# ollieeknight/mgatk2

Measured on AMD Instinct MI355X. Metric: chrM reads piled-up/sec (whole node) at 200M reads × 10k cells; bit-exact counts, higher is better.
Workload: dtype u32

## Files before the change

include/mgpileup.h:

```cpp
#ifndef MGPILEUP_H
#define MGPILEUP_H

#include <stdint.h>

#ifdef __cplusplus
extern "C" {
#endif

#define MGP_ABI_VERSION 7

#define MGP_OK               0
#define MGP_E_INVALID      (-1)
#define MGP_E_HIP          (-2)
#define MGP_E_OOM          (-3)
#define MGP_E_UNSORTED     (-4)
#define MGP_E_BADREAD      (-5)
#define MGP_E_SPAN         (-6)
#define MGP_E_STATE        (-7)
#define MGP_E_COMM         (-8)

#define MGP_DEDUP_NONE        0
#define MGP_DEDUP_START       1
#define MGP_DEDUP_START_FRAG  2

// ... 404 lines not shown
int  mgp_louvain(int device, int64_t n_vertices, int64_t n_edges, const int32_t *edge_i, const int32_t *edge_j,
                 const int32_t *edge_w, double resolution, int32_t max_levels, int32_t max_passes,
                 int32_t *labels , int64_t *n_communities, double *modularity,
                 uint64_t *sums , int32_t *n_levels, int64_t *levels );
int  mgp_windows(mgp_ctx *ctx, int32_t *n_windows, int32_t *window_width);
int  mgp_copy_wait(mgp_ctx *ctx);
int  mgp_set_cell_range(mgp_ctx *ctx, int32_t cell_lo, int32_t cell_hi);
int  mgp_push_batch16(mgp_ctx *ctx, const mgp_batch16 *batch);
int  mgp_set_streaming(mgp_ctx *ctx, int on);
int  mgp_stream_info(mgp_ctx *ctx, int64_t *segments, int32_t *last_streamed);
int  mgp_finish(mgp_ctx *ctx, mgp_result *out);

int  mgp_kernel_times(mgp_ctx *ctx, int last_runs, float *ms, int max_n, int *n_out, char *names, int names_len);
int  mgp_set_stage_timing(mgp_ctx *ctx, int all_stages);

int  mgp_comm_unique_id(uint8_t *out128);
int  mgp_comm_init(mgp_ctx *ctx, const uint8_t *uid128, int nranks, int rank);

int  mgp_synth_generate(mgp_ctx *ctx, const mgp_synth_params *p);
int  mgp_download_inputs(mgp_ctx *ctx, int32_t *start, int32_t *bc, int32_t *tlen,
                         uint16_t *flag, uint8_t *mapq, uint32_t *span,
                         uint64_t *rec_off, uint8_t *payload);

int  mgp_bgzf_inflate(int device, const uint8_t *src, int64_t src_bytes, int64_t n_blocks,
                      const uint64_t *coff, const uint32_t *clen, const uint32_t *isize, const uint64_t *out_off,
                      uint8_t *out, int64_t out_bytes, int32_t *status );
typedef struct mgp_inflater mgp_inflater;
int  mgp_inflater_create(int device, int64_t max_src_bytes, int64_t max_out_bytes, mgp_inflater **out);
void mgp_inflater_destroy(mgp_inflater *inflater);
int  mgp_inflater_run(void *inflater, const uint8_t *src, int64_t src_bytes, int64_t n_blocks,
                      const uint64_t *coff, const uint32_t *clen, const uint32_t *isize, const uint64_t *out_off,
                      uint8_t *out, int64_t out_bytes, int32_t *status);
int  mgp_inflater_times(mgp_inflater *inflater, double *ms3, int64_t *calls, int64_t *blocks);
void *mgp_inflater_host_alloc(int64_t bytes);
void  mgp_inflater_host_release(void *p);

int  mgp_zlib_inflate(int device, const uint8_t *src, int64_t src_bytes, int64_t n_streams,
                      const uint64_t *coff, const uint32_t *clen, const uint32_t *isize, const uint64_t *out_off,
                      uint8_t *out, int64_t out_bytes, int32_t *status );
int  mgp_open_table(int hip_device, int32_t n_cells, int32_t mito_len, mgp_ctx **out);
typedef struct mgp_table_chunks {
    int64_t        n_cols;
    int32_t        chunk_rows, chunk_cols;
    int32_t        col_chunk_lo, col_chunk_hi;
    int32_t        first_cell;
    int32_t        reserved;
    const uint8_t *src;
    int64_t        src_bytes;
    const int64_t *chunk_bytes;
    const uint8_t *raw;
    int64_t        n_saturated;
    double         ms[3];
} mgp_table_chunks;
int  mgp_table_load(mgp_ctx *table, mgp_table_chunks *job);
int  mgp_table_load_planes(mgp_ctx *table, mgp_table_chunks *job);
int  mgp_table_check(int32_t n_cells, int32_t mito_len, const mgp_table_chunks *job, int planes);
int  mgp_table_ready(mgp_ctx *table);

#ifdef __cplusplus
}
#endif
#endif
```

mgatk2_amd/csrc/mgp_inflate.hip:

```cpp
#include <hip/hip_runtime.h>

#include <cstring>
#include <string>
#include <vector>

#include "../../include/mgpileup.h"
#include "mgp_host.h"
#include "mgp_inflate_core.h"

namespace {

using namespace mgp_inflate;

struct DeviceWave {
    __device__ uint32_t lane() const { return threadIdx.x; }
    __device__ uint32_t width() const { return 64; }
    __device__ bool leader() const { return threadIdx.x == 0; }
    __device__ void sync() const { __syncthreads(); }
};

__global__ __launch_bounds__(64) void inflate_blocks(const uint8_t* __restrict__ src, const uint64_t* __restrict__ coff,
                                                     const uint32_t* __restrict__ clen,
                                                     const uint32_t* __restrict__ isize,
                                                     const uint64_t* __restrict__ out_off, uint8_t* __restrict__ out,
                                                     int32_t* __restrict__ status, uint32_t n_blocks) {
    __shared__ Scratch sc;
    __shared__ alignas(16) uint8_t win[kMaxIsize];
    const uint32_t b = blockIdx.x;
    if (b >= n_blocks) return;
    const DeviceWave w;
    const uint32_t n = isize[b];
    const int32_t st = inflate(w, src + coff[b], clen[b], win, n, &sc);
    if (st == ST_OK) flush(w, win, n, out + out_off[b]);
    if (w.leader()) status[b] = st;
}

struct Args {
    const uint8_t* src;
    int64_t src_bytes, n_blocks;
    const uint64_t* coff;
    const uint32_t* clen;
    const uint32_t* isize;
    const uint64_t* out_off;
    uint8_t* out;
    int64_t out_bytes;
    int32_t* status;
};

int check_args(const char* who, const Args& a) {
    const std::string w(who);
    if (a.n_blocks < 0 || a.src_bytes < 0 || a.out_bytes < 0) return set_err(MGP_E_INVALID, w + ": negative count");
    if (a.n_blocks > 0x7FFFFFFF) return set_err(MGP_E_INVALID, w + ": more than 2^31 - 1 blocks in one call");
    if (a.n_blocks && (!a.coff || !a.clen || !a.isize || !a.out_off || !a.status))
        return set_err(MGP_E_INVALID, w + ": null array");
    if ((a.src_bytes && !a.src) || (a.out_bytes && !a.out)) return set_err(MGP_E_INVALID, w + ": null buffer");
    uint64_t end = 0;
    for (int64_t i = 0; i < a.n_blocks; ++i) {
        const std::string at = " (block " + std::to_string(i) + ")";
        if (a.isize[i] > kMaxIsize) return set_err(MGP_E_INVALID, w + ": isize above 65536" + at);
        if (a.coff[i] > (uint64_t)a.src_bytes || a.clen[i] > (uint64_t)a.src_bytes - a.coff[i])
            return set_err(MGP_E_INVALID, w + ": compressed range outside src" + at);
        if (a.out_off[i] > (uint64_t)a.out_bytes || a.isize[i] > (uint64_t)a.out_bytes - a.out_off[i])
            return set_err(MGP_E_INVALID, w + ": output range outside out" + at);
        if (a.out_off[i] < end) return set_err(MGP_E_INVALID, w + ": output ranges unsorted or overlapping" + at);
        end = a.out_off[i] + a.isize[i];
    }
// ... 125 lines not shown
    if (inf->s) (void)hipStreamSynchronize(inf->s);
    delete inf;
}

int mgp_inflater_run(void* inflater, const uint8_t* src, int64_t src_bytes, int64_t n_blocks, const uint64_t* coff,
                     const uint32_t* clen, const uint32_t* isize, const uint64_t* out_off, uint8_t* out,
                     int64_t out_bytes, int32_t* status) {
    if (!inflater) return set_err(MGP_E_INVALID, "mgp_inflater_run: null inflater");
    const Args a{src, src_bytes, n_blocks, coff, clen, isize, out_off, out, out_bytes, status};
    return inflater_run(static_cast<mgp_inflater*>(inflater), "mgp_inflater_run", a);
}

int mgp_bgzf_inflate(int device, const uint8_t* src, int64_t src_bytes, int64_t n_blocks, const uint64_t* coff,
                     const uint32_t* clen, const uint32_t* isize, const uint64_t* out_off, uint8_t* out,
                     int64_t out_bytes, int32_t* status) {
    const Args a{src, src_bytes, n_blocks, coff, clen, isize, out_off, out, out_bytes, status};
    MGP_TRY(check_args("mgp_bgzf_inflate", a));
    if (n_blocks == 0) return MGP_OK;
    mgp_inflater* inf = nullptr;
    MGP_TRY(inflater_create(device, src_bytes, out_bytes, &inf));
    const int rc = inflater_run(inf, "mgp_bgzf_inflate", a);
    mgp_inflater_destroy(inf);
    return rc;
}

int mgp_inflater_times(mgp_inflater* inf, double* ms3, int64_t* calls, int64_t* blocks) {
    if (!inf || !ms3) return set_err(MGP_E_INVALID, "mgp_inflater_times: null argument");
    for (int k = 0; k < 3; ++k) ms3[k] = inf->ms[k];
    if (calls) *calls = inf->calls;
    if (blocks) *blocks = inf->blocks;
    return MGP_OK;
}

void* mgp_inflater_host_alloc(int64_t bytes) {
    void* p = nullptr;
    return mgp_host_alloc(bytes, &p) == MGP_OK ? p : nullptr;
}
void mgp_inflater_host_release(void* p) { (void)mgp_host_free(p); }

}
```

mgatk2_amd/csrc/mgp_inflate_core.h:

```cpp
#pragma once
#include <stdint.h>

#if defined(__HIPCC__) || defined(__CUDACC__)
#define MGPI_HD __host__ __device__
#else
#define MGPI_HD
#endif

namespace mgp_inflate {

enum : int32_t { ST_OK = 0, ST_INVALID = 1, ST_SIZE = 2, ST_CHECK = 3 };

constexpr uint32_t kMaxIsize = 65536;
constexpr uint32_t kRing = 65536, kHalf = 32768;
constexpr uint32_t kAdlerMod = 65521;
constexpr uint32_t kMaxLanes = 64;
constexpr uint32_t kInWin = 4096;
constexpr uint32_t kLitBits = 10, kDistBits = 8, kClBits = 7;
constexpr uint32_t kMaxLit = 288, kMaxDist = 32, kMaxCl = 19;

struct Huff {
    uint16_t count[16];
    uint16_t first[16];
    uint16_t offs[16];
    uint16_t sorted[kMaxLit];
};

struct Scratch {
    alignas(16) uint8_t inwin[kInWin];
    uint16_t lit_tab[1u << kLitBits];
    uint16_t dist_tab[1u << kDistBits];
    uint16_t cl_tab[1u << kClBits];
    Huff lit, dist, cl;
    uint8_t lens[kMaxLit + kMaxDist];
    uint8_t cl_lens[kMaxCl + 1];
    uint32_t red[2 * kMaxLanes];
};

struct HostWave {
    MGPI_HD uint32_t lane() const { return 0; }
    MGPI_HD uint32_t width() const { return 1; }
    MGPI_HD bool leader() const { return true; }
    MGPI_HD void sync() const {}
};

struct Bits {
    const uint8_t* src;
    uint32_t clen;
    uint64_t bitbuf = 0;
    uint32_t bitcnt = 0;
    uint32_t ip = 0;
    uint32_t wbase = 0, wend = 0;
};

template <class W>
MGPI_HD inline void fill_window(const W& w, Bits& b, Scratch* s) {
    w.sync();
    b.wbase = b.ip;
    b.wend = b.ip + kInWin;
    for (uint32_t i = w.lane(); i < kInWin; i += w.width()) {
        const uint32_t g = b.wbase + i;
        s->inwin[i] = g < b.clen ? b.src[g] : (uint8_t)0;
    }
    w.sync();
}

template <class W>
MGPI_HD inline void refill(const W& w, Bits& b, Scratch* s) {
    for (int k = 0; k < 2; ++k) {
        if (b.bitcnt > 32 || b.ip >= b.clen) return;
        if (b.ip >= b.wend) fill_window(w, b, s);
        const uint32_t o = b.ip - b.wbase;
        const uint32_t word = (uint32_t)s->inwin[o] | (uint32_t)s->inwin[o + 1] << 8 | (uint32_t)s->inwin[o + 2] << 16 |
                              (uint32_t)s->inwin[o + 3] << 24;
        const uint32_t left = b.clen - b.ip;
        const uint32_t nb = left < 4 ? left : 4;
        b.bitbuf |= (uint64_t)word << b.bitcnt;
        b.bitcnt += 8 * nb;
        b.ip += nb;
    }
}

MGPI_HD inline uint32_t peek(const Bits& b, uint32_t n) { return (uint32_t)(b.bitbuf & ((1ull << n) - 1)); }
MGPI_HD inline void drop(Bits& b, uint32_t n) {
    b.bitbuf >>= n;
    b.bitcnt -= n;
}

MGPI_HD inline uint32_t bitrev(uint32_t v, uint32_t n) {
    uint32_t r = 0;
    for (uint32_t i = 0; i < 15; ++i) {
        if (i < n) r |= ((v >> i) & 1u) << (n - 1 - i);
    }
    return r;
}

template <class W>
MGPI_HD inline int32_t build(const W& w, const uint8_t* lens, uint32_t nsym, uint32_t cap, bool is_codes, Huff* h,
                             uint16_t* tab, uint32_t bits) {
    if (nsym > cap) nsym = cap;
    const uint32_t tsize = 1u << bits;
    w.sync();
    for (uint32_t l = w.lane(); l < 16; l += w.width()) {
        uint32_t c = 0;
        for (uint32_t i = 0; i < nsym; ++i) c += (lens[i] & 15u) == l;
        h->count[l] = (uint16_t)c;
    }
    for (uint32_t i = w.lane(); i < tsize; i += w.width()) tab[i] = 0;
    w.sync();
    uint32_t maxlen = 0;
    int32_t left = 1;
    bool over = false;
    for (uint32_t l = 1; l < 16; ++l) {
        const uint32_t c = h->count[l];
        if (c) maxlen = l;
        left <<= 1;
        left -= (int32_t)c;
        if (left < 0) {
            over = true;
            left = 0;
        }
    }
    if (over) return ST_INVALID;
    if (maxlen == 0) return is_codes ? ST_INVALID : ST_OK;
    if (left > 0 && (is_codes || maxlen != 1)) return ST_INVALID;
    if (w.leader()) {
        uint32_t code = 0, off = 0;
        h->first[0] = 0;
        h->offs[0] = 0;
        for (uint32_t l = 1; l < 16; ++l) {
            code = (code + h->count[l - 1] * (l > 1)) << 1;
            h->first[l] = (uint16_t)code;
            h->offs[l] = (uint16_t)off;
            off += h->count[l];
        }
    }
    w.sync();
    for (uint32_t l = 1 + w.lane(); l < 16; l += w.width()) {
        uint32_t k = h->offs[l];
        const uint32_t end = k + h->count[l];
        for (uint32_t i = 0; i < nsym; ++i)
            if ((lens[i] & 15u) == l && k < end && k < kMaxLit) h->sorted[k++] = (uint16_t)i;
    }
    w.sync();
    const uint32_t nused = nsym - h->count[0];
    for (uint32_t j = w.lane(); j < nused && j < kMaxLit; j += w.width()) {
        const uint32_t sym = h->sorted[j];
        const uint32_t l = sym < nsym ? (lens[sym] & 15u) : 0;
        if (l == 0 || l > bits) continue;
        const uint32_t code = (uint32_t)h->first[l] + (j - h->offs[l]);
        const uint16_t e = (uint16_t)(sym << 4 | l);
        for (uint32_t k = bitrev(code, l) & (tsize - 1); k < tsize; k += 1u << l) tab[k] = e;
    }
    w.sync();
    return ST_OK;
}

MGPI_HD inline int32_t decode(const Bits& b, const Huff* h, const uint16_t* tab, uint32_t bits, uint32_t* sym,
                              uint32_t* len) {
    const uint32_t e = tab[peek(b, bits)];
    if (e & 15u) {
        *sym = e >> 4;
        *len = e & 15u;
        return ST_OK;
    }
    uint32_t code = 0, first = 0, index = 0;
    uint64_t v = b.bitbuf;
    for (uint32_t l = 1; l < 16; ++l) {
        code |= (uint32_t)(v & 1);
        v >>= 1;
        const uint32_t c = h->count[l];
        if (code < first + c) {
            const uint32_t k = index + (code - first);
            if (k >= kMaxLit) return ST_INVALID;
            *sym = h->sorted[k];
            *len = l;
            return ST_OK;
        }
        index += c;
        first = (first + c) << 1;
        code <<= 1;
    }
    return ST_INVALID;
}

MGPI_HD inline uint32_t len_base(uint32_t s) {
    return s < 8 ? 3 + s : s == 28 ? 258 : 3 + ((4 + (s & 3)) << ((s >> 2) - 1));
}
MGPI_HD inline uint32_t len_extra(uint32_t s) { return s < 8 || s == 28 ? 0 : (s >> 2) - 1; }
MGPI_HD inline uint32_t dist_base(uint32_t s) {
    return s < 4 ? 1 + s : 1 + ((2 + (s & 1)) << ((s >> 1) - 1));
}
MGPI_HD inline uint32_t dist_extra(uint32_t s) { return s < 4 ? 0 : (s >> 1) - 1; }

template <class W>
MGPI_HD inline void fixed_lens(const W& w, Scratch* s) {
    w.sync();
    for (uint32_t i = w.lane(); i < kMaxLit + kMaxDist; i += w.width())
        s->lens[i] = (uint8_t)(i < 144 ? 8 : i < 256 ? 9 : i < 280 ? 7 : i < 288 ? 8 : 5);
}

template <class W>
MGPI_HD inline int32_t dynamic_header(const W& w, Bits& b, Scratch* s, uint32_t* nlen_out, uint32_t* ndist_out) {
    constexpr uint64_t order_lo = 16ull | 17ull << 5 | 18ull << 10 | 0ull << 15 | 8ull << 20 | 7ull << 25 | 9ull << 30 |
                                  6ull << 35 | 10ull << 40 | 5ull << 45 | 11ull << 50 | 4ull << 55;
    constexpr uint64_t order_hi = 12ull | 3ull << 5 | 13ull << 10 | 2ull << 15 | 14ull << 20 | 1ull << 25 | 15ull << 30;
    refill(w, b, s);
    if (b.bitcnt < 14) return ST_SIZE;
    const uint32_t nlen = peek(b, 5) + 257;
    drop(b, 5);
    const uint32_t ndist = peek(b, 5) + 1;
    drop(b, 5);
    const uint32_t ncode = peek(b, 4) + 4;
    drop(b, 4);
    if (nlen > 286 || ndist > 30) return ST_INVALID;
    w.sync();
    for (uint32_t i = 0; i < kMaxCl; ++i) {
        uint32_t v = 0;
        if (i < ncode) {
            refill(w, b, s);
            if (b.bitcnt < 3) return ST_SIZE;
            v = peek(b, 3);
            drop(b, 3);
        }
        const uint32_t at = (uint32_t)((i < 12 ? order_lo >> (5 * i) : order_hi >> (5 * (i - 12))) & 31u);
        if (w.leader() && at < kMaxCl) s->cl_lens[at] = (uint8_t)v;
    }
    int32_t rc = build(w, s->cl_lens, kMaxCl, kMaxCl, true, &s->cl, s->cl_tab, kClBits);
    if (rc != ST_OK) return rc;
    const uint32_t total = nlen + ndist;
    uint32_t have = 0, prev = 0;
    for (uint32_t step = 0; step < kMaxLit + kMaxDist && have < total; ++step) {
        refill(w, b, s);
        uint32_t sym, len;
        if (decode(b, &s->cl, s->cl_tab, kClBits, &sym, &len) != ST_OK) return ST_INVALID;
        if (len > b.bitcnt) return ST_SIZE;
        drop(b, len);
        uint32_t rep = 1, val = sym;
        if (sym >= 16) {
            const uint32_t eb = sym == 16 ? 2 : sym == 17 ? 3 : 7;
            if (sym > 18) return ST_INVALID;
            if (b.bitcnt < eb) return ST_SIZE;
            if (sym == 16 && have == 0) return ST_INVALID;
            rep = (sym == 16 ? 3 : sym == 17 ? 3 : 11) + peek(b, eb);
            drop(b, eb);
            val = sym == 16 ? prev : 0;
            if (have + rep > total) return ST_INVALID;
        }
        if (w.leader())
            for (uint32_t k = 0; k < rep; ++k) {
                const uint32_t i = have + k;
                const uint32_t at = i < nlen ? i : kMaxLit + (i - nlen);
                if (at < kMaxLit + kMaxDist) s->lens[at] = (uint8_t)val;
            }
        have += rep;
        prev = val;
    }
    if (have != total) return ST_INVALID;
    w.sync();
    if (s->lens[256] == 0) return ST_INVALID;
    *nlen_out = nlen;
    *ndist_out = ndist;
    return ST_OK;
}

template <class W>
MGPI_HD inline int32_t inflate(const W& w, const uint8_t* src, uint32_t clen, uint8_t* win, uint32_t isize, Scratch* s) {
    if (isize > kMaxIsize || clen >= 0x80000000u) return ST_INVALID;
    Bits b;
    b.src = src;
    b.clen = clen;
    uint32_t op = 0;
    uint64_t budget = 8ull * clen + 64;
    bool final_seen = false;
    while (!final_seen) {
        if (budget-- == 0) return ST_INVALID;
        refill(w, b, s);
        if (b.bitcnt < 3) return ST_SIZE;
        final_seen = peek(b, 1) != 0;
        const uint32_t type = peek(b, 3) >> 1;
        drop(b, 3);
        if (type == 3) return ST_INVALID;
        if (type == 0) {
            drop(b, b.bitcnt & 7);
            refill(w, b, s);
            if (b.bitcnt < 32) return ST_SIZE;
            const uint32_t len = peek(b, 16);
            drop(b, 16);
            const uint32_t nlen = peek(b, 16);
            drop(b, 16);
            if ((len ^ 0xFFFFu) != nlen) return ST_INVALID;
            const uint32_t pos = b.ip - (b.bitcnt >> 3);
            if (len > clen - pos) return ST_SIZE;
            if (len > isize - op) return ST_SIZE;
            w.sync();
            for (uint32_t i = w.lane(); i < len; i += w.width()) win[op + i] = src[pos + i];
            w.sync();
            op += len;
            b.bitbuf = 0;
            b.bitcnt = 0;
            b.ip = pos + len;
            b.wbase = b.wend = b.ip;
            continue;
        }
        uint32_t nlen = kMaxLit, ndist = kMaxDist;
        if (type == 1) {
            fixed_lens(w, s);
        } else {
            const int32_t rc = dynamic_header(w, b, s, &nlen, &ndist);
            if (rc != ST_OK) return rc;
        }
        int32_t rc = build(w, s->lens, nlen, kMaxLit, false, &s->lit, s->lit_tab, kLitBits);
        if (rc != ST_OK) return rc;
        rc = build(w, s->lens + kMaxLit, ndist, kMaxDist, false, &s->dist, s->dist_tab, kDistBits);
        if (rc != ST_OK) return rc;
        bool end_of_block = false;
        while (!end_of_block) {
            if (budget-- == 0) return ST_INVALID;
            refill(w, b, s);
            uint32_t sym, len;
            if (decode(b, &s->lit, s->lit_tab, kLitBits, &sym, &len) != ST_OK) return ST_INVALID;
            if (len > b.bitcnt) return ST_SIZE;
            drop(b, len);
            if (sym < 256) {
                if (op >= isize) return ST_SIZE;
                if (w.leader()) win[op] = (uint8_t)sym;
                ++op;
                continue;
            }
            if (sym == 256) {
                end_of_block = true;
                continue;
            }
            if (sym >= 286) return ST_INVALID;
            const uint32_t ls = sym - 257;
            const uint32_t le = len_extra(ls);
            if (b.bitcnt < le) return ST_SIZE;
            const uint32_t mlen = len_base(ls) + peek(b, le);
            drop(b, le);
            refill(w, b, s);
            uint32_t dsym, dlen;
            if (decode(b, &s->dist, s->dist_tab, kDistBits, &dsym, &dlen) != ST_OK) return ST_INVALID;
            if (dlen > b.bitcnt) return ST_SIZE;
            drop(b, dlen);
            if (dsym >= 30) return ST_INVALID;
            const uint32_t de = dist_extra(dsym);
            if (b.bitcnt < de) return ST_SIZE;
            const uint32_t dist = dist_base(dsym) + peek(b, de);
            drop(b, de);
            if (dist > op) return ST_INVALID;
            if (mlen > isize - op) return ST_SIZE;
            w.sync();
            const uint32_t from = op - dist;
            if (dist >= mlen) {
                for (uint32_t i = w.lane(); i < mlen; i += w.width()) win[op + i] = win[from + i];
            } else {
                for (uint32_t i = w.lane(); i < mlen; i += w.width()) win[op + i] = win[from + i % dist];
            }
            w.sync();
            op += mlen;
        }
    }
    w.sync();
    return op == isize ? ST_OK : ST_SIZE;
}

template <class W>
MGPI_HD inline void flush(const W& w, const uint8_t* win, uint32_t n, uint8_t* dst) {
    const uint32_t mis = (uint32_t)((4u - ((uintptr_t)dst & 3u)) & 3u);
    const uint32_t head = mis < n ? mis : n;
    const uint32_t words = (n - head) >> 2;
    const uint32_t tail0 = head + 4 * words;
    for (uint32_t i = w.lane(); i < head; i += w.width()) dst[i] = win[i];
    uint32_t* d32 = reinterpret_cast<uint32_t*>(dst + head);
    for (uint32_t k = w.lane(); k < words; k += w.width()) {
        const uint8_t* p = win + head + 4 * k;
        d32[k] = (uint32_t)p[0] | (uint32_t)p[1] << 8 | (uint32_t)p[2] << 16 | (uint32_t)p[3] << 24;
    }
    for (uint32_t i = tail0 + w.lane(); i < n; i += w.width()) dst[i] = win[i];
}

template <class W>
MGPI_HD inline void flush_ring(const W& w, const uint8_t* ring, uint32_t from, uint32_t n, uint8_t* dst, Scratch* s,
                               uint32_t* a, uint32_t* b) {
    if (n == 0) return;
    w.sync();
    const uint8_t* p = ring + (from & (kRing - 1));
    flush(w, p, n, dst + from);
    uint64_t s1 = 0, s2 = 0;
    for (uint32_t i = w.lane(); i < n; i += w.width()) {
        const uint64_t d = p[i];
        s1 += d;
        s2 += (uint64_t)(n - i) * d;
    }
    const uint32_t l = w.lane() < kMaxLanes ? w.lane() : kMaxLanes - 1;
    s->red[2 * l] = (uint32_t)(s1 % kAdlerMod);
    s->red[2 * l + 1] = (uint32_t)(s2 % kAdlerMod);
    w.sync();
    uint64_t t1 = 0, t2 = 0;
    const uint32_t nl = w.width() < kMaxLanes ? w.width() : kMaxLanes;
    for (uint32_t k = 0; k < nl; ++k) {
        t1 += s->red[2 * k];
        t2 += s->red[2 * k + 1];
    }
    const uint64_t a0 = *a;
    *a = (uint32_t)((a0 + t1) % kAdlerMod);
    *b = (uint32_t)((*b + (uint64_t)n * a0 + t2) % kAdlerMod);
    w.sync();
}

template <class W>
MGPI_HD inline int32_t inflate_zlib(const W& w, const uint8_t* src, uint32_t clen, uint8_t* ring, uint8_t* dst,
// ... 35 lines not shown
                w.sync();
                for (uint32_t i = w.lane(); i < n; i += w.width()) ring[(op + i) & (kRing - 1)] = b.src[pos + i];
                op += n;
                pos += n;
                left -= n;
                if (op - flushed == kHalf) {
                    flush_ring(w, ring, flushed, kHalf, dst, s, &ad_a, &ad_b);
                    flushed += kHalf;
                }
            }
            w.sync();
            b.bitbuf = 0;
            b.bitcnt = 0;
            b.ip = pos;
            b.wbase = b.wend = b.ip;
            continue;
        }
        uint32_t nlen = kMaxLit, ndist = kMaxDist;
        if (type == 1) {
            fixed_lens(w, s);
        } else {
            const int32_t rc = dynamic_header(w, b, s, &nlen, &ndist);
            if (rc != ST_OK) return rc;
        }
        int32_t rc = build(w, s->lens, nlen, kMaxLit, false, &s->lit, s->lit_tab, kLitBits);
        if (rc != ST_OK) return rc;
        rc = build(w, s->lens + kMaxLit, ndist, kMaxDist, false, &s->dist, s->dist_tab, kDistBits);
        if (rc != ST_OK) return rc;
        bool end_of_block = false;
        while (!end_of_block) {
            if (budget-- == 0) return ST_INVALID;
            refill(w, b, s);
            uint32_t sym, len;
            if (decode(b, &s->lit, s->lit_tab, kLitBits, &sym, &len) != ST_OK) return ST_INVALID;
            if (len > b.bitcnt) return ST_SIZE;
            drop(b, len);
            if (sym < 256) {
                if (op >= isize) return ST_SIZE;
                if (w.leader()) ring[op & (kRing - 1)] = (uint8_t)sym;
                ++op;
            } else if (sym == 256) {
                end_of_block = true;
                continue;
            } else {
                if (sym >= 286) return ST_INVALID;
                const uint32_t ls = sym - 257;
                const uint32_t le = len_extra(ls);
                if (b.bitcnt < le) return ST_SIZE;
                const uint32_t mlen = len_base(ls) + peek(b, le);
                drop(b, le);
                refill(w, b, s);
                uint32_t dsym, dlen;
                if (decode(b, &s->dist, s->dist_tab, kDistBits, &dsym, &dlen) != ST_OK) return ST_INVALID;
                if (dlen > b.bitcnt) return ST_SIZE;
                drop(b, dlen);
                if (dsym >= 30) return ST_INVALID;
                const uint32_t de = dist_extra(dsym);
                if (b.bitcnt < de) return ST_SIZE;
                const uint32_t dist = dist_base(dsym) + peek(b, de);
                drop(b, de);
                if (dist > op) return ST_INVALID;
                if (mlen > isize - op) return ST_SIZE;
                w.sync();
                const uint32_t from = op - dist;
                if (dist >= mlen) {
                    for (uint32_t i = w.lane(); i < mlen; i += w.width())
                        ring[(op + i) & (kRing - 1)] = ring[(from + i) & (kRing - 1)];
                } else {
                    for (uint32_t i = w.lane(); i < mlen; i += w.width())
                        ring[(op + i) & (kRing - 1)] = ring[(from + i % dist) & (kRing - 1)];
                }
                w.sync();
                op += mlen;
            }
            if (op - flushed >= kHalf) {
                flush_ring(w, ring, flushed, kHalf, dst, s, &ad_a, &ad_b);
                flushed += kHalf;
            }
        }
    }
    if (op != isize) return ST_SIZE;
    flush_ring(w, ring, flushed, op - flushed, dst, s, &ad_a, &ad_b);
    const uint32_t pos = b.ip - (b.bitcnt >> 3);
    if (b.clen - pos < 4) return ST_SIZE;
    const uint8_t* t = b.src + pos;
    const uint32_t want = (uint32_t)t[0] << 24 | (uint32_t)t[1] << 16 | (uint32_t)t[2] << 8 | (uint32_t)t[3];
// ... 6 lines not shown
```

mgatk2_amd/engine.py:

```python

from __future__ import annotations

import ctypes as C
from dataclasses import dataclass
from pathlib import Path

import numpy as np

from .exceptions import BAMFormatError, BAMReadError, InvalidInputError, ProcessingError
from .synth import ReadSoA

import os

LIB_PATH = Path(os.environ.get("MGP_LIB") or Path(__file__).resolve().parent / "_lib" / "libmgpileup.so")

MGP_OK = 0
MGP_E_INVALID = -1
MGP_E_HIP = -2
MGP_E_OOM = -3
MGP_E_UNSORTED = -4
MGP_E_BADREAD = -5
MGP_E_SPAN = -6
MGP_E_STATE = -7
MGP_E_COMM = -8

DEDUP_MODES = {"none": 0, "alignment_start": 1, "alignment_and_fragment_length": 2}

ABI_SYMBOLS = (
    "mgp_abi_version", "mgp_last_error", "mgp_device_count", "mgp_open", "mgp_close", "mgp_host_alloc",
    "mgp_host_free", "mgp_push_batch", "mgp_reset", "mgp_resident", "mgp_run", "mgp_sync", "mgp_fetch",
    "mgp_finish", "mgp_kernel_times", "mgp_comm_unique_id", "mgp_comm_init", "mgp_synth_generate",
    "mgp_download_inputs", "mgp_set_stage_timing", "mgp_fetch_cells", "mgp_fetch_rows16", "mgp_windows",
    "mgp_stream_info", "mgp_set_streaming", "mgp_set_rows16_target", "mgp_copy_wait", "mgp_set_cell_range",
    "mgp_push_batch16", "mgp_txt_gz_run", "mgp_txt_gz_fetch", "mgp_txt_gz_rows", "mgp_set_rows_target",
    "mgp_h5_tiles_run", "mgp_h5_tiles_fetch", "mgp_h5_tiles_rows", "mgp_variant_moments_run", "mgp_variant_dev2_run",
    "mgp_allele_freq_run", "mgp_variant_moments_rows", "mgp_variant_dev2_rows", "mgp_allele_freq_rows",
    "mgp_cell_coverage_run", "mgp_position_coverage_run", "mgp_position_depth_hist_run",
    "mgp_position_depth_next_run", "mgp_cell_coverage_rows", "mgp_position_coverage_rows",
    "mgp_position_depth_hist_rows", "mgp_position_depth_next_rows", "mgp_pair_dist", "mgp_hclust_dist", "mgp_hclust",
    "mgp_knn", "mgp_snn", "mgp_louvain", "mgp_bgzf_inflate", "mgp_inflater_create", "mgp_inflater_destroy",
    "mgp_inflater_run", "mgp_inflater_host_alloc", "mgp_inflater_host_release", "mgp_inflater_times",
    "mgp_zlib_inflate", "mgp_open_table", "mgp_table_load", "mgp_table_load_planes", "mgp_table_check",
    "mgp_table_ready", "mgp_group_moments_run", "mgp_rows_group_moments", "mgp_rank_sums",
)
ABI_VERSION = 7
CFG_KEEP_TN5 = 0x1
CFG_STREAM = 0x2


class mgp_config(C.Structure):
    _fields_ = [
        ("min_baseq", C.c_int32),
        ("min_mapq", C.c_int32),
        ("min_dist_from_end", C.c_int32),
        ("dedup_mode", C.c_int32),
        ("max_strand_bias", C.c_double),
        ("min_reads", C.c_int32),
        ("n_cells", C.c_int32),
        ("mito_len", C.c_int32),
        ("flags", C.c_int32),
        ("reserve_reads", C.c_int64),
        ("reserve_payload", C.c_int64),
    ]


class mgp_batch16(C.Structure):
    _fields_ = [
        ("n_reads", C.c_int64),
        ("bc", C.c_void_p),
        ("abs_tlen", C.c_void_p),
        ("flag", C.c_void_p),
        ("mapq", C.c_void_p),
        ("payload", C.c_void_p),
        ("payload_bytes", C.c_int64),
# ... 251 lines not shown
        ),
        "mgp_rows_group_moments": (
            [C.c_int, vp, vp, i32, i32, C.POINTER(mgp_variant_job), vp, i32, i32, C.POINTER(mgp_group_moments)], C.c_int
        ),
        "mgp_cell_coverage_run": ([vp, C.POINTER(mgp_variant_job), C.POINTER(mgp_cell_coverage)], C.c_int),
        "mgp_position_coverage_run": ([vp, C.POINTER(mgp_variant_job), C.POINTER(mgp_position_coverage)], C.c_int),
        "mgp_position_depth_hist_run": ([vp, C.POINTER(mgp_variant_job), i32, vp, vp], C.c_int),
        "mgp_position_depth_next_run": ([vp, C.POINTER(mgp_variant_job), vp, vp, vp], C.c_int),
        "mgp_cell_coverage_rows": (
            [C.c_int, vp, i32, i32, C.POINTER(mgp_variant_job), C.POINTER(mgp_cell_coverage)], C.c_int
        ),
        "mgp_position_coverage_rows": (
            [C.c_int, vp, vp, vp, i32, i32, C.POINTER(mgp_variant_job), C.POINTER(mgp_position_coverage)], C.c_int
        ),
        "mgp_position_depth_hist_rows": ([C.c_int, vp, i32, i32, C.POINTER(mgp_variant_job), i32, vp, vp], C.c_int),
        "mgp_position_depth_next_rows": ([C.c_int, vp, i32, i32, C.POINTER(mgp_variant_job), vp, vp, vp], C.c_int),
        "mgp_pair_dist": ([C.c_int, vp, i64, i64, vp], C.c_int),
        "mgp_hclust_dist": ([C.c_int, vp, i64, vp, vp, vp], C.c_int),
        "mgp_hclust": ([C.c_int, vp, i64, i64, vp, vp, vp, vp], C.c_int),
        "mgp_knn": ([C.c_int, vp, i64, i64, i32, vp, vp], C.c_int),
        "mgp_rank_sums": ([C.c_int, vp, i64, i64, vp, i32, vp, vp, vp], C.c_int),
        "mgp_snn": ([C.c_int, vp, i64, i32, i32, i64, C.POINTER(i64), vp, vp, vp], C.c_int),
        "mgp_louvain": (
            [C.c_int, i64, i64, vp, vp, vp, C.c_double, i32, i32, vp, C.POINTER(i64), C.POINTER(C.c_double), vp,
             C.POINTER(i32), vp], C.c_int
        ),
        "mgp_bgzf_inflate": ([C.c_int, vp, i64, i64, vp, vp, vp, vp, vp, i64, vp], C.c_int),
        "mgp_inflater_create": ([C.c_int, i64, i64, C.POINTER(vp)], C.c_int),
        "mgp_inflater_destroy": ([vp], None),
        "mgp_inflater_run": ([vp, vp, i64, i64, vp, vp, vp, vp, vp, i64, vp], C.c_int),
        "mgp_inflater_host_alloc": ([i64], vp),
        "mgp_inflater_host_release": ([vp], None),
        "mgp_inflater_times": ([vp, C.POINTER(C.c_double), C.POINTER(i64), C.POINTER(i64)], C.c_int),
        "mgp_zlib_inflate": ([C.c_int, vp, i64, i64, vp, vp, vp, vp, vp, i64, vp], C.c_int),
        "mgp_open_table": ([C.c_int, i32, i32, C.POINTER(vp)], C.c_int),
        "mgp_table_load": ([vp, C.POINTER(mgp_table_chunks)], C.c_int),
        "mgp_table_load_planes": ([vp, C.POINTER(mgp_table_chunks)], C.c_int),
        "mgp_table_check": ([i32, i32, C.POINTER(mgp_table_chunks), C.c_int], C.c_int),
        "mgp_table_ready": ([vp], C.c_int),
    }
    for name, (args, res) in sig.items():
        fn = getattr(lib, name)
        fn.argtypes = args
        fn.restype = res
    if lib.mgp_abi_version() != ABI_VERSION:
        raise ProcessingError("libmgpileup ABI version mismatch")
    if path is None:
        _lib = lib
    return lib


def _raise(code: int, what: str):
    lib = load_library()
    msg = (lib.mgp_last_error() or b"").decode(errors="replace")
    text = f"{what}: {msg} (code {code})"
    if code == MGP_E_INVALID or code == MGP_E_SPAN:
        raise InvalidInputError(text)
    if code == MGP_E_UNSORTED:
        raise BAMFormatError("<resident reads>", text)
    if code == MGP_E_BADREAD:
        raise BAMReadError("<resident reads>", text)
    raise ProcessingError(text)


def _ck(code: int, what: str):
    if code != MGP_OK:
# ... 521 lines not shown
                                     _ptr(out["pos"]), _ptr(out["ties"])), "mgp_rank_sums")
    return out


LOUVAIN_MAX_VERTICES = 1 << 20
LOUVAIN_MAX_EDGES = 1 << 30
LOUVAIN_MAX_WEIGHT = 1 << 20
LOUVAIN_MAX_LEVELS = 64
LOUVAIN_MAX_PASSES = 1 << 16
LOUVAIN_WAVE_ROW = 64
LOUVAIN_LDS_ROW = 2048


def graph_louvain(n: int, i, j, wq, resolution: float = 1.0, max_levels: int = 32, max_passes: int = 64,
                  device: int = 0) -> dict:
    i, j, wq = (np.ascontiguousarray(a, np.int32).reshape(-1) for a in (i, j, wq))
    if not i.size == j.size == wq.size:
        raise InvalidInputError("i, j and wq have one entry per edge")
    n, ne = int(n), int(i.size)
    ok = 0 <= n <= LOUVAIN_MAX_VERTICES and 1 <= int(max_levels) <= LOUVAIN_MAX_LEVELS
    labels = np.zeros(n if ok else 0, np.int32)
    levels = np.zeros((int(max_levels) if ok else 1, 4), np.int64)
    sums = np.zeros(4, np.uint64)
    nc, nl, q = C.c_int64(0), C.c_int32(0), C.c_double(0.0)
    _ck(load_library().mgp_louvain(int(device), n, ne, _ptr(i), _ptr(j), _ptr(wq), float(resolution), int(max_levels),
                                   int(max_passes), _ptr(labels), C.byref(nc), C.byref(q), _ptr(sums), C.byref(nl),
                                   _ptr(levels)), "mgp_louvain")
    return {"labels": labels, "n_communities": int(nc.value), "modularity": float(q.value), "m2": int(sums[0]),
            "internal": int(sums[1]), "b": (int(sums[2]) << 64) | int(sums[3]),
            "levels": [tuple(int(x) for x in row) for row in levels[: nl.value]]}


INFLATE_MAX_ISIZE = 65536


def _inflate_args(src, coff, clen, isize, out_off, out):
    src = np.ascontiguousarray(np.frombuffer(src, np.uint8) if isinstance(src, (bytes, bytearray)) else src, np.uint8)
    coff = np.ascontiguousarray(coff, np.uint64)
    clen = np.ascontiguousarray(clen, np.uint32)
    isize = np.ascontiguousarray(isize, np.uint32)
    out_off = np.ascontiguousarray(out_off, np.uint64)
    n = int(coff.shape[0])
    if not (clen.shape[0] == isize.shape[0] == out_off.shape[0] == n):
        raise InvalidInputError("coff, clen, isize and out_off have one entry per block")
    if out.dtype != np.uint8 or not out.flags.c_contiguous or not out.flags.writeable:
        raise InvalidInputError("out is a writable contiguous uint8 array")
    status = np.full(n, -1, np.int32)
    return (_ptr(src), int(src.shape[0]), n, _ptr(coff), _ptr(clen), _ptr(isize), _ptr(out_off), _ptr(out),
            int(out.shape[0]), _ptr(status)), status, (src, coff, clen, isize, out_off)


def inflate_bgzf(src, coff, clen, isize, out_off, out: np.ndarray, device: int = 0) -> np.ndarray:
    args, status, keep = _inflate_args(src, coff, clen, isize, out_off, out)
    _ck(load_library().mgp_bgzf_inflate(int(device), *args), "mgp_bgzf_inflate")
    del keep
    return status


def inflate_zlib(src, coff, clen, isize, out_off, out: np.ndarray, device: int = 0) -> np.ndarray:
    args, status, keep = _inflate_args(src, coff, clen, isize, out_off, out)
    _ck(load_library().mgp_zlib_inflate(int(device), *args), "mgp_zlib_inflate")
    del keep
    return status


class Inflater:
# ... 433 lines not shown
```

Measured before the change: 777.8 million.

## Decode BGZF blocks through a 33KB LDS ring to raise inflate occupancy

The GPU inflate kernel now decodes into a 33KB shared-memory ring buffer and streams 1KB units to global output, replacing the full 64KB LDS window. Together with a smaller input window, this lets four workgroups share a CU's LDS, where before far fewer fit. Workgroup barriers become wave-level barriers, and scalar values are broadcast with readfirstlane. Literals are batched up to four per write, and input words are prefetched with aligned loads. The costs are more frequent flush synchronisation and more complex ring wraparound logic, plus a new geometry query API.

```diff
diff --git a/include/mgpileup.h b/include/mgpileup.h
--- a/include/mgpileup.h
+++ b/include/mgpileup.h
@@ -460,6 +460,7 @@
                       const uint64_t *coff, const uint32_t *clen, const uint32_t *isize, const uint64_t *out_off,
                       uint8_t *out, int64_t out_bytes, int32_t *status);
 int  mgp_inflater_times(mgp_inflater *inflater, double *ms3, int64_t *calls, int64_t *blocks);
+int  mgp_inflate_geometry(uint32_t *v4);
 void *mgp_inflater_host_alloc(int64_t bytes);
 void  mgp_inflater_host_release(void *p);
 
diff --git a/mgatk2_amd/csrc/mgp_inflate.hip b/mgatk2_amd/csrc/mgp_inflate.hip
--- a/mgatk2_amd/csrc/mgp_inflate.hip
+++ b/mgatk2_amd/csrc/mgp_inflate.hip
@@ -16,7 +16,12 @@
     __device__ uint32_t lane() const { return threadIdx.x; }
     __device__ uint32_t width() const { return 64; }
     __device__ bool leader() const { return threadIdx.x == 0; }
-    __device__ void sync() const { __syncthreads(); }
+    __device__ uint32_t uni(uint32_t v) const { return (uint32_t)__builtin_amdgcn_readfirstlane((int)v); }
+    __device__ void sync() const {
+        __builtin_amdgcn_fence(__ATOMIC_RELEASE, "wavefront");
+        __builtin_amdgcn_wave_barrier();
+        __builtin_amdgcn_fence(__ATOMIC_ACQUIRE, "wavefront");
+    }
 };
 
 __global__ __launch_bounds__(64) void inflate_blocks(const uint8_t* __restrict__ src, const uint64_t* __restrict__ coff,
@@ -24,14 +29,13 @@
                                                      const uint32_t* __restrict__ isize,
                                                      const uint64_t* __restrict__ out_off, uint8_t* __restrict__ out,
                                                      int32_t* __restrict__ status, uint32_t n_blocks) {
-    __shared__ Scratch sc;
-    __shared__ alignas(16) uint8_t win[kMaxIsize];
+    __shared__ RingScratch sc;
+    __shared__ alignas(16) uint8_t ring[kBRing];
+    static_assert(sizeof(RingScratch) + kBRing <= 160 * 1024 / 4, "four workgroups to a CU's LDS");
     const uint32_t b = blockIdx.x;
     if (b >= n_blocks) return;
     const DeviceWave w;
-    const uint32_t n = isize[b];
-    const int32_t st = inflate(w, src + coff[b], clen[b], win, n, &sc);
-    if (st == ST_OK) flush(w, win, n, out + out_off[b]);
+    const int32_t st = inflate_ring(w, src + coff[b], clen[b], ring, out + out_off[b], isize[b], &sc);
     if (w.leader()) status[b] = st;
 }
 
@@ -223,6 +227,15 @@
     return MGP_OK;
 }
 
+int mgp_inflate_geometry(uint32_t* v4) {
+    if (!v4) return set_err(MGP_E_INVALID, "mgp_inflate_geometry: null argument");
+    v4[0] = kBRing;
+    v4[1] = kBUnit;
+    v4[2] = kBInWin;
+    v4[3] = kLitStep;
+    return MGP_OK;
+}
+
 void* mgp_inflater_host_alloc(int64_t bytes) {
     void* p = nullptr;
     return mgp_host_alloc(bytes, &p) == MGP_OK ? p : nullptr;
diff --git a/mgatk2_amd/csrc/mgp_inflate_core.h b/mgatk2_amd/csrc/mgp_inflate_core.h
--- a/mgatk2_amd/csrc/mgp_inflate_core.h
+++ b/mgatk2_amd/csrc/mgp_inflate_core.h
@@ -18,6 +18,9 @@
 constexpr uint32_t kInWin = 4096;
 constexpr uint32_t kLitBits = 10, kDistBits = 8, kClBits = 7;
 constexpr uint32_t kMaxLit = 288, kMaxDist = 32, kMaxCl = 19;
+constexpr uint32_t kBUnit = 1024, kBRing = 32768 + kBUnit, kBInWin = 1024, kLitStep = 4;
+static_assert(kBRing % kBUnit == 0 && kBUnit >= 258 + kLitStep && kBUnit <= 32768, "inflate_ring's invariants");
+static_assert(kMaxIsize < 2 * kBRing, "a block passes the ring's seam once at most");
 
 struct Huff {
     uint16_t count[16];
@@ -26,16 +29,20 @@
     uint16_t sorted[kMaxLit];
 };
 
-struct Scratch {
-    alignas(16) uint8_t inwin[kInWin];
+template <uint32_t InWin, uint32_t Red>
+struct ScratchT {
+    static constexpr uint32_t kWin = InWin;
+    alignas(16) uint8_t inwin[InWin];
     uint16_t lit_tab[1u << kLitBits];
     uint16_t dist_tab[1u << kDistBits];
     uint16_t cl_tab[1u << kClBits];
     Huff lit, dist, cl;
     uint8_t lens[kMaxLit + kMaxDist];
     uint8_t cl_lens[kMaxCl + 1];
-    uint32_t red[2 * kMaxLanes];
+    uint32_t red[Red];
 };
+using Scratch = ScratchT<kInWin, 2 * kMaxLanes>;
+using RingScratch = ScratchT<kBInWin, 2>;
 
 struct HostWave {
     MGPI_HD uint32_t lane() const { return 0; }
@@ -43,6 +50,15 @@
     MGPI_HD bool leader() const { return true; }
     MGPI_HD void sync() const {}
 };
+
+template <class W>
+MGPI_HD inline auto uni(const W& w, uint32_t v, int) -> decltype(w.uni(v)) {
+    return w.uni(v);
+}
+template <class W>
+MGPI_HD inline uint32_t uni(const W&, uint32_t v, long) {
+    return v;
+}
 
 struct Bits {
     const uint8_t* src;
@@ -51,33 +67,42 @@
     uint32_t bitcnt = 0;
     uint32_t ip = 0;
     uint32_t wbase = 0, wend = 0;
+    uint32_t ahead = 0;
 };
 
-template <class W>
-MGPI_HD inline void fill_window(const W& w, Bits& b, Scratch* s) {
+template <class S>
+MGPI_HD inline uint32_t window_word(const S* s, uint32_t o) {
+    uint32_t v;
+    __builtin_memcpy(&v, __builtin_assume_aligned(s->inwin + o, 4), 4);
+    return v;
+}
+
+template <class W, class S>
+MGPI_HD inline void fill_window(const W& w, Bits& b, S* s) {
     w.sync();
     b.wbase = b.ip;
-    b.wend = b.ip + kInWin;
-    for (uint32_t i = w.lane(); i < kInWin; i += w.width()) {
+    b.wend = b.ip + S::kWin;
+    for (uint32_t i = w.lane(); i < S::kWin; i += w.width()) {
         const uint32_t g = b.wbase + i;
         s->inwin[i] = g < b.clen ? b.src[g] : (uint8_t)0;
     }
     w.sync();
 }
 
-template <class W>
-MGPI_HD inline void refill(const W& w, Bits& b, Scratch* s) {
+template <class W, class S>
+MGPI_HD inline void refill(const W& w, Bits& b, S* s) {
     for (int k = 0; k < 2; ++k) {
         if (b.bitcnt > 32 || b.ip >= b.clen) return;
-        if (b.ip >= b.wend) fill_window(w, b, s);
-        const uint32_t o = b.ip - b.wbase;
-        const uint32_t word = (uint32_t)s->inwin[o] | (uint32_t)s->inwin[o + 1] << 8 | (uint32_t)s->inwin[o + 2] << 16 |
-                              (uint32_t)s->inwin[o + 3] << 24;
+        if (b.ip >= b.wend) {
+            fill_window(w, b, s);
+            b.ahead = window_word(s, 0);
+        }
         const uint32_t left = b.clen - b.ip;
         const uint32_t nb = left < 4 ? left : 4;
-        b.bitbuf |= (uint64_t)word << b.bitcnt;
+        b.bitbuf |= (uint64_t)uni(w, b.ahead, 0) << b.bitcnt;
         b.bitcnt += 8 * nb;
         b.ip += nb;
+        if (b.ip < b.wend && b.ip < b.clen) b.ahead = window_word(s, b.ip - b.wbase);
     }
 }
 
@@ -112,7 +137,7 @@
     int32_t left = 1;
     bool over = false;
     for (uint32_t l = 1; l < 16; ++l) {
-        const uint32_t c = h->count[l];
+        const uint32_t c = uni(w, h->count[l], 0);
         if (c) maxlen = l;
         left <<= 1;
         left -= (int32_t)c;
@@ -156,24 +181,26 @@
     return ST_OK;
 }
 
-MGPI_HD inline int32_t decode(const Bits& b, const Huff* h, const uint16_t* tab, uint32_t bits, uint32_t* sym,
+template <class W>
+MGPI_HD inline int32_t decode(const W& w, const Bits& b, const Huff* h, const uint16_t* tab, uint32_t bits, uint32_t* sym,
                               uint32_t* len) {
-    const uint32_t e = tab[peek(b, bits)];
+    const uint32_t e = uni(w, tab[peek(b, bits)], 0);
     if (e & 15u) {
         *sym = e >> 4;
         *len = e & 15u;
         return ST_OK;
     }
+    asm volatile("" ::: "memory");
     uint32_t code = 0, first = 0, index = 0;
     uint64_t v = b.bitbuf;
     for (uint32_t l = 1; l < 16; ++l) {
         code |= (uint32_t)(v & 1);
         v >>= 1;
-        const uint32_t c = h->count[l];
+        const uint32_t c = uni(w, h->count[l], 0);
         if (code < first + c) {
             const uint32_t k = index + (code - first);
             if (k >= kMaxLit) return ST_INVALID;
-            *sym = h->sorted[k];
+            *sym = uni(w, h->sorted[k], 0);
             *len = l;
             return ST_OK;
         }
@@ -193,15 +220,15 @@
 }
 MGPI_HD inline uint32_t dist_extra(uint32_t s) { return s < 4 ? 0 : (s >> 1) - 1; }
 
-template <class W>
-MGPI_HD inline void fixed_lens(const W& w, Scratch* s) {
+template <class W, class S>
+MGPI_HD inline void fixed_lens(const W& w, S* s) {
     w.sync();
     for (uint32_t i = w.lane(); i < kMaxLit + kMaxDist; i += w.width())
         s->lens[i] = (uint8_t)(i < 144 ? 8 : i < 256 ? 9 : i < 280 ? 7 : i < 288 ? 8 : 5);
 }
 
-template <class W>
-MGPI_HD inline int32_t dynamic_header(const W& w, Bits& b, Scratch* s, uint32_t* nlen_out, uint32_t* ndist_out) {
+template <class W, class S>
+MGPI_HD inline int32_t dynamic_header(const W& w, Bits& b, S* s, uint32_t* nlen_out, uint32_t* ndist_out) {
     constexpr uint64_t order_lo = 16ull | 17ull << 5 | 18ull << 10 | 0ull << 15 | 8ull << 20 | 7ull << 25 | 9ull << 30 |
                                   6ull << 35 | 10ull << 40 | 5ull << 45 | 11ull << 50 | 4ull << 55;
     constexpr uint64_t order_hi = 12ull | 3ull << 5 | 13ull << 10 | 2ull << 15 | 14ull << 20 | 1ull << 25 | 15ull << 30;
@@ -233,7 +260,7 @@
     for (uint32_t step = 0; step < kMaxLit + kMaxDist && have < total; ++step) {
         refill(w, b, s);
         uint32_t sym, len;
-        if (decode(b, &s->cl, s->cl_tab, kClBits, &sym, &len) != ST_OK) return ST_INVALID;
+        if (decode(w, b, &s->cl, s->cl_tab, kClBits, &sym, &len) != ST_OK) return ST_INVALID;
         if (len > b.bitcnt) return ST_SIZE;
         drop(b, len);
         uint32_t rep = 1, val = sym;
@@ -258,7 +285,7 @@
     }
     if (have != total) return ST_INVALID;
     w.sync();
-    if (s->lens[256] == 0) return ST_INVALID;
+    if (uni(w, s->lens[256], 0) == 0) return ST_INVALID;
     *nlen_out = nlen;
     *ndist_out = ndist;
     return ST_OK;
@@ -319,7 +346,7 @@
             if (budget-- == 0) return ST_INVALID;
             refill(w, b, s);
             uint32_t sym, len;
-            if (decode(b, &s->lit, s->lit_tab, kLitBits, &sym, &len) != ST_OK) return ST_INVALID;
+            if (decode(w, b, &s->lit, s->lit_tab, kLitBits, &sym, &len) != ST_OK) return ST_INVALID;
             if (len > b.bitcnt) return ST_SIZE;
             drop(b, len);
             if (sym < 256) {
@@ -340,7 +367,7 @@
             drop(b, le);
             refill(w, b, s);
             uint32_t dsym, dlen;
-            if (decode(b, &s->dist, s->dist_tab, kDistBits, &dsym, &dlen) != ST_OK) return ST_INVALID;
+            if (decode(w, b, &s->dist, s->dist_tab, kDistBits, &dsym, &dlen) != ST_OK) return ST_INVALID;
             if (dlen > b.bitcnt) return ST_SIZE;
             drop(b, dlen);
             if (dsym >= 30) return ST_INVALID;
@@ -378,6 +405,149 @@
         d32[k] = (uint32_t)p[0] | (uint32_t)p[1] << 8 | (uint32_t)p[2] << 16 | (uint32_t)p[3] << 24;
     }
     for (uint32_t i = tail0 + w.lane(); i < n; i += w.width()) dst[i] = win[i];
+}
+
+MGPI_HD inline uint32_t ring_at(uint32_t x) { return x >= kBRing ? x - kBRing : x; }
+
+template <class W, class S>
+MGPI_HD inline int32_t inflate_ring(const W& w, const uint8_t* src, uint32_t clen, uint8_t* ring, uint8_t* dst,
+                                    uint32_t isize, S* s) {
+    if (isize > kMaxIsize || clen >= 0x80000000u) return ST_INVALID;
+    Bits b;
+    b.src = src;
+    b.clen = clen;
+    uint32_t op = 0, flushed = 0, rp = 0, fp = 0;
+    uint64_t budget = 8ull * clen + 64;
+    bool final_seen = false;
+    while (!final_seen) {
+        if (budget-- == 0) return ST_INVALID;
+        refill(w, b, s);
+        if (b.bitcnt < 3) return ST_SIZE;
+        final_seen = peek(b, 1) != 0;
+        const uint32_t type = peek(b, 3) >> 1;
+        drop(b, 3);
+        if (type == 3) return ST_INVALID;
+        if (type == 0) {
+            drop(b, b.bitcnt & 7);
+            refill(w, b, s);
+            if (b.bitcnt < 32) return ST_SIZE;
+            const uint32_t len = peek(b, 16);
+            drop(b, 16);
+            const uint32_t nlen = peek(b, 16);
+            drop(b, 16);
+            if ((len ^ 0xFFFFu) != nlen) return ST_INVALID;
+            uint32_t pos = b.ip - (b.bitcnt >> 3);
+            if (len > clen - pos) return ST_SIZE;
+            if (len > isize - op) return ST_SIZE;
+            for (uint32_t left = len; left;) {
+                const uint32_t room = kBUnit - (op - flushed), n = left < room ? left : room;
+                w.sync();
+                for (uint32_t i = w.lane(); i < n; i += w.width()) ring[rp + i] = src[pos + i];
+                op += n;
+                pos += n;
+                left -= n;
+                rp = ring_at(rp + n);
+                if (op - flushed == kBUnit) {
+                    w.sync();
+                    flush(w, ring + fp, kBUnit, dst + flushed);
+                    w.sync();
+                    flushed += kBUnit;
+                    fp = ring_at(fp + kBUnit);
+                }
+            }
+            w.sync();
+            b.bitbuf = 0;
+            b.bitcnt = 0;
+            b.ip = pos;
+            b.wbase = b.wend = b.ip;
+            continue;
+        }
+        uint32_t nlen = kMaxLit, ndist = kMaxDist;
+        if (type == 1) {
+            fixed_lens(w, s);
+        } else {
+            const int32_t rc = dynamic_header(w, b, s, &nlen, &ndist);
+            if (rc != ST_OK) return rc;
+        }
+        int32_t rc = build(w, s->lens, nlen, kMaxLit, false, &s->lit, s->lit_tab, kLitBits);
+        if (rc != ST_OK) return rc;
+        rc = build(w, s->lens + kMaxLit, ndist, kMaxDist, false, &s->dist, s->dist_tab, kDistBits);
+        if (rc != ST_OK) return rc;
+        bool end_of_block = false;
+        while (!end_of_block) {
+            if (budget-- == 0) return ST_INVALID;
+            refill(w, b, s);
+            uint32_t sym, len, nlit = 0, lits = 0;
+            for (;;) {
+                if (decode(w, b, &s->lit, s->lit_tab, kLitBits, &sym, &len) != ST_OK) return ST_INVALID;
+                if (len > b.bitcnt) return ST_SIZE;
+                if (sym >= 256) break;
+                drop(b, len);
+                if (nlit >= isize - op) return ST_SIZE;
+                lits |= sym << (8 * nlit);
+                ++nlit;
+                if (nlit == kLitStep || b.bitcnt < 15) break;
+            }
+            if (nlit) {
+                for (uint32_t i = w.lane(); i < nlit; i += w.width())
+                    ring[ring_at(rp + i)] = (uint8_t)(lits >> (8 * i));
+                op += nlit;
+                rp = ring_at(rp + nlit);
+            }
+            if (sym == 256) {
+                drop(b, len);
+                end_of_block = true;
+            } else if (sym > 256) {
+                if (sym >= 286) return ST_INVALID;
+                drop(b, len);
+                if (nlit) refill(w, b, s);
+                const uint32_t ls = sym - 257;
+                const uint32_t le = len_extra(ls);
+                if (b.bitcnt < le) return ST_SIZE;
+                const uint32_t mlen = len_base(ls) + peek(b, le);
+                drop(b, le);
+                refill(w, b, s);
+                uint32_t dsym, dlen;
+                if (decode(w, b, &s->dist, s->dist_tab, kDistBits, &dsym, &dlen) != ST_OK) return ST_INVALID;
+                if (dlen > b.bitcnt) return ST_SIZE;
+                drop(b, dlen);
+                if (dsym >= 30) return ST_INVALID;
+                const uint32_t de = dist_extra(dsym);
+                if (b.bitcnt < de) return ST_SIZE;
+                const uint32_t dist = dist_base(dsym) + peek(b, de);
+                drop(b, de);
+                if (dist > op) return ST_INVALID;
+                if (mlen > isize - op) return ST_SIZE;
+                w.sync();
+                const uint32_t from = rp >= dist ? rp - dist : rp + kBRing - dist;
+                if (dist >= mlen) {
+                    for (uint32_t i = w.lane(); i < mlen; i += w.width()) ring[ring_at(rp + i)] = ring[ring_at(from + i)];
+                } else {
+                    uint32_t r = w.lane() % dist;
+                    const uint32_t step = w.width() % dist;
+                    for (uint32_t i = w.lane(); i < mlen; i += w.width()) {
+                        ring[ring_at(rp + i)] = ring[ring_at(from + r)];
+                        r += step;
+                        if (r >= dist) r -= dist;
+                    }
+                }
+                w.sync();
+                op += mlen;
+                rp = ring_at(rp + mlen);
+            }
+            if (op - flushed >= kBUnit) {
+                w.sync();
+                flush(w, ring + fp, kBUnit, dst + flushed);
+                w.sync();
+                flushed += kBUnit;
+                fp = ring_at(fp + kBUnit);
+            }
+        }
+    }
+    if (op != isize) return ST_SIZE;
+    w.sync();
+    flush(w, ring + fp, op - flushed, dst + flushed);
+    return ST_OK;
 }
 
 template <class W>
@@ -479,7 +649,7 @@
             if (budget-- == 0) return ST_INVALID;
             refill(w, b, s);
             uint32_t sym, len;
-            if (decode(b, &s->lit, s->lit_tab, kLitBits, &sym, &len) != ST_OK) return ST_INVALID;
+            if (decode(w, b, &s->lit, s->lit_tab, kLitBits, &sym, &len) != ST_OK) return ST_INVALID;
             if (len > b.bitcnt) return ST_SIZE;
             drop(b, len);
             if (sym < 256) {
@@ -498,7 +668,7 @@
                 drop(b, le);
                 refill(w, b, s);
                 uint32_t dsym, dlen;
-                if (decode(b, &s->dist, s->dist_tab, kDistBits, &dsym, &dlen) != ST_OK) return ST_INVALID;
+                if (decode(w, b, &s->dist, s->dist_tab, kDistBits, &dsym, &dlen) != ST_OK) return ST_INVALID;
                 if (dlen > b.bitcnt) return ST_SIZE;
                 drop(b, dlen);
                 if (dsym >= 30) return ST_INVALID;
diff --git a/mgatk2_amd/engine.py b/mgatk2_amd/engine.py
--- a/mgatk2_amd/engine.py
+++ b/mgatk2_amd/engine.py
@@ -40,6 +40,7 @@
     "mgp_position_depth_hist_rows", "mgp_position_depth_next_rows", "mgp_pair_dist", "mgp_hclust_dist", "mgp_hclust",
     "mgp_knn", "mgp_snn", "mgp_louvain", "mgp_bgzf_inflate", "mgp_inflater_create", "mgp_inflater_destroy",
     "mgp_inflater_run", "mgp_inflater_host_alloc", "mgp_inflater_host_release", "mgp_inflater_times",
+    "mgp_inflate_geometry",
     "mgp_zlib_inflate", "mgp_open_table", "mgp_table_load", "mgp_table_load_planes", "mgp_table_check",
     "mgp_table_ready", "mgp_group_moments_run", "mgp_rows_group_moments", "mgp_rank_sums",
 )
@@ -357,6 +358,7 @@
         "mgp_inflater_host_alloc": ([i64], vp),
         "mgp_inflater_host_release": ([vp], None),
         "mgp_inflater_times": ([vp, C.POINTER(C.c_double), C.POINTER(i64), C.POINTER(i64)], C.c_int),
+        "mgp_inflate_geometry": ([C.POINTER(C.c_uint32)], C.c_int),
         "mgp_zlib_inflate": ([C.c_int, vp, i64, i64, vp, vp, vp, vp, vp, i64, vp], C.c_int),
         "mgp_open_table": ([C.c_int, i32, i32, C.POINTER(vp)], C.c_int),
         "mgp_table_load": ([vp, C.POINTER(mgp_table_chunks)], C.c_int),
@@ -944,6 +946,12 @@
 
 
 INFLATE_MAX_ISIZE = 65536
+
+
+def inflate_geometry() -> dict:
+    v = (C.c_uint32 * 4)()
+    _ck(load_library().mgp_inflate_geometry(v), "mgp_inflate_geometry")
+    return {"ring": int(v[0]), "unit": int(v[1]), "in_window": int(v[2]), "lit_step": int(v[3])}
 
 
 def _inflate_args(src, coff, clen, isize, out_off, out):
```

Measured after the change: 776.7 million (median of 2 runs). No clear change (-0.1%).
